# zsyOAOA/ResShift

Measured on AMD Instinct MI355X. Metric: images/sec (1x3x64x64 LR -> 3x256x256, 15-step ResShift sampling loop incl. VQ encode/decode), higher is better.
Workload: dtype f16x2 encoder + UNet (hi+lo fp16 pairs, 3 MFMAs per product: fp32-class) + f16 decoder (parity policy); 1 GPU; realsr_swinunet_realesrgan256: batch 32/GPU x 1 GPU, 1x3x64x64 LR -> 3x256x256, 15 steps, random-init weights; precision_policy=parity, parallelism=dp1 (batch sharded, one RCCL weight broadcast, no data-path collective)

## Files before the change

### include/resshift_hip.h

```cpp
#ifndef RESSHIFT_HIP_H
#define RESSHIFT_HIP_H
#include <stddef.h>
#include <stdint.h>

#ifdef __cplusplus
extern "C" {
#endif

#define RS_PREC_F16 0
#define RS_PREC_F32 1
#define RS_PREC_SPLIT 2
#define RS_MAX_LEVELS 8
#define RS_MAX_STEPS 64
#define RS_MAX_ROWS 64

typedef struct rs_engine rs_engine;

typedef struct rs_unet_config {
    int image_size, in_channels, model_channels, out_channels;
    int n_levels;
    int channel_mult[RS_MAX_LEVELS];
    int num_res_blocks[RS_MAX_LEVELS];
    int n_attn_res;
    int attention_resolutions[RS_MAX_LEVELS];
// ... 136 lines not shown
int rs_op_groupnorm(const void* x, void* y, const float* gamma_host, const float* beta_host, const float* film_dev, int B, int HW,
                    int C, int groups, float eps, int act, int prec, void* stream);
int rs_op_window_attention(const void* qkv, void* out, const float* bias_table_host , int B, int H, int W,
                           int heads, int shift, int prec, void* stream);
int rs_op_window_attention_qkv(const void* x, const void* wqkv_dev, const float* bqkv_dev, const void* wproj_dev, const float* bproj_dev,
                               const void* res, void* out, const float* table_host, int B, int H, int W, int heads, int shift, void* stream);
int rs_op_window_attention_qkv_split(const void* x, const void* wqkv_dev, const float* bqkv_dev, const void* wproj_dev, const float* bproj_dev,
                                     const void* res, void* out, const float* table_host, const float* xcoef_dev, int B, int H, int W, int heads,
                                     int shift, void* stream);
int rs_op_ae_flash_attention(const void* q, const void* k, const void* vt, const float* bv_dev, void* o, int nz, int T, int C, void* stream);
int rs_op_ae_flash_attention_split(const void* q, const void* k, const void* vt, const float* bv_dev, void* o, int nz, int T, int C, void* stream);
int rs_op_swin_mlp(const void* x, const void* w1_dev, const float* b1_dev, const void* w2_dev, const float* b2_dev, const void* res, void* y,
                   int M, int E, int HD, void* stream);
int rs_op_swin_mlp_split(const void* x, const void* w1_dev, const float* b1_dev, const void* w2_dev, const float* b2_dev, const void* res, void* y,
                         int M, int E, int HD, void* stream);
int rs_op_swin_mlp_split_unembed(const void* x, const float* xcoef_dev, const void* w1_dev, const float* b1_dev, const void* w2cat_dev, const float* bcat_dev,
                                 void* y, int M, int HW, int E, int HD, int NO, void* stream);
int rs_op_softmax_rows(const float* s, void* out, long long nrows, int ncols, int out_prec, void* stream);
int rs_op_vq(const float* z, const float* codebook_dev, float* zq, int32_t* idx, long long N, int NE, int D, void* stream);
int rs_op_nchw_to_nhwc(const float* in, void* out, int B, int C, int HW, int out_prec, void* stream);
int rs_op_nhwc_to_nchw(const void* in, float* out, int B, int C, int HW, int in_prec, void* stream);
int rs_op_convert(const void* src, int src_prec, void* dst, int dst_prec, int C, long long npix, void* stream);

#ifdef __cplusplus
}
#endif
#endif
```

### resshift_amd/_lib.py

```python
from __future__ import annotations

import ctypes as C
import os

import torch

HERE = os.path.dirname(os.path.abspath(__file__))
LIB_PATH = os.environ.get("RESSHIFT_HIP_LIB") or os.path.join(HERE, "libresshift_hip.so")

RS_PREC_F16 = 0
RS_PREC_F32 = 1
RS_PREC_SPLIT = 2
RS_MAX_LEVELS = 8
RS_MAX_STEPS = 64
RS_MAX_ROWS = 64


class UNetConfig(C.Structure):
    _fields_ = [
        ("image_size", C.c_int), ("in_channels", C.c_int), ("model_channels", C.c_int), ("out_channels", C.c_int),
        ("n_levels", C.c_int),
        ("channel_mult", C.c_int * RS_MAX_LEVELS),
        ("num_res_blocks", C.c_int * RS_MAX_LEVELS),
        ("n_attn_res", C.c_int),
# ... 110 lines not shown
    "rs_debug_fetch_rows": (_I, [_P, _I, _I, _I, _P, _P]),
    "rs_op_conv2d": (_I, [_P, _P, _P, _P, _P, _P] + [_I] * 18 + [_P]),
    "rs_op_conv2d_bench": (_I, [_P, _P, _P, _P, _P] + [_I] * 16 + [C.POINTER(C.c_float), _P]),
    "rs_op_conv3x3_halo_stats_px": (_I, [_I, _I, _I, _I, _I, _I]),
    "rs_op_conv3x3_halo": (_I, [_P, _P, _I, _P, _P, _P, _P, _I, _I, _I, _I, _I, _I, _P, _P]),
    "rs_op_conv3x3_wino": (_I, [_P, _P, _I, _P, _P, _P, _P, _I, _I, _I, _I, _I, _P, _I, C.POINTER(C.c_float), _P]),
    "rs_op_gemm_nt": (_I, [_P, _P, _P, _P, _I, _I, _I, _I, _F, _I, _I, _P]),
    "rs_op_groupnorm": (_I, [_P, _P, _P, _P, _P, _I, _I, _I, _I, _F, _I, _I, _P]),
    "rs_op_window_attention": (_I, [_P, _P, _P, _I, _I, _I, _I, _I, _I, _P]),
    "rs_op_window_attention_qkv": (_I, [_P, _P, _P, _P, _P, _P, _P, _P, _I, _I, _I, _I, _I, _P]),
    "rs_op_window_attention_qkv_split": (_I, [_P, _P, _P, _P, _P, _P, _P, _P, _P, _I, _I, _I, _I, _I, _P]),
    "rs_op_swin_mlp": (_I, [_P, _P, _P, _P, _P, _P, _P, _I, _I, _I, _P]),
    "rs_op_ae_flash_attention": (_I, [_P, _P, _P, _P, _P, _I, _I, _I, _P]),
    "rs_op_ae_flash_attention_split": (_I, [_P, _P, _P, _P, _P, _I, _I, _I, _P]),
    "rs_op_swin_mlp_split": (_I, [_P, _P, _P, _P, _P, _P, _P, _I, _I, _I, _P]),
    "rs_op_swin_mlp_split_unembed": (_I, [_P, _P, _P, _P, _P, _P, _P, _I, _I, _I, _I, _I, _P]),
    "rs_op_softmax_rows": (_I, [_P, _P, _LL, _I, _I, _P]),
    "rs_op_vq": (_I, [_P, _P, _P, _P, _LL, _I, _I, _P]),
    "rs_op_nchw_to_nhwc": (_I, [_P, _P, _I, _I, _I, _I, _P]),
    "rs_op_nhwc_to_nchw": (_I, [_P, _P, _I, _I, _I, _I, _P]),
    "rs_op_convert": (_I, [_P, _I, _P, _I, _I, _LL, _P]),
}

_lib = None


def load() -> C.CDLL:
    global _lib
    if _lib is not None:
        return _lib
# ... 91 lines not shown
```

### resshift_amd/csrc/engine.hip

```cpp
#include "common.h"
#include "../../include/resshift_hip.h"
#include <dlfcn.h>
#include <algorithm>
#include <array>
#include <cmath>
#include <cstdio>
#include <cstring>
#include <functional>
#include <map>
#include <string>
#include <unordered_map>
#include <vector>

extern "C" {
int rs_igemm_launch(const IGemmParams* p, int in_dt, int out_dt, int nz, hipStream_t st);
int rs_igemm_splitk_plan(int M, int Cout, int Ktot, int in_dt);
int rs_igemm4_pick(const IGemmParams* p, int in_dt, int out_dt, int nz, int* TW, int* BC);
int rs_igemm4_plan(const IGemmParams* p, int in_dt, int out_dt, int nz, int* TW, int* BC, int* SEG, int* SK);
int rs_igemm4_stats_px(const IGemmParams* p, int in_dt);
int rs_wino_plan(const IGemmParams* p, int in_dt, int out_dt, int nz);
int rs_wino_launch(const IGemmParams* p, hipStream_t st);
size_t rs_wino_weight_bytes(int Cin, int Cout);
float rs_wino_pack(const float* w_ref, int Cin, int Cout, void* dst);
int rs_wino_stats_px();
// ... 2588 lines not shown
    return rc;
}

int rs_op_swin_mlp(const void* x, const void* w1_dev, const float* b1_dev, const void* w2_dev, const float* b2_dev, const void* res, void* y,
                   int M, int E, int HD, void* stream) {
    const int rc = rs_swin_mlp_launch(x, w1_dev, b1_dev, w2_dev, b2_dev, res, y, M, E, E, E, E, HD, nullptr, 0, nullptr, 0, (hipStream_t)stream);
    if (rc) fail("swin_mlp launch rejected the shape (fp16, E = 192, HD = 768 only)");
    return rc;
}
int rs_op_swin_mlp_split(const void* x, const void* w1_dev, const float* b1_dev, const void* w2_dev, const float* b2_dev, const void* res, void* y,
                         int M, int E, int HD, void* stream) {
    const int rc = rs_swin_mlp_split_launch(x, w1_dev, b1_dev, w2_dev, b2_dev, res, y, M, E, E, E, E, HD, nullptr, 0, nullptr, 0, nullptr, (hipStream_t)stream);
    if (rc) fail("swin_mlp_split launch rejected the shape (split storage, E = 192, HD = 768 only)");
    return rc;
}
int rs_op_swin_mlp_split_unembed(const void* x, const float* xcoef_dev, const void* w1_dev, const float* b1_dev, const void* w2cat_dev, const float* bcat_dev,
                                 void* y, int M, int HW, int E, int HD, int NO, void* stream) {
    const int rc = rs_swin_mlp_split_launch_n(x, w1_dev, b1_dev, w2cat_dev, bcat_dev, nullptr, y, M, E, 0, NO, E, HD, NO, xcoef_dev, HW, nullptr, 0, nullptr,
                                              (hipStream_t)stream);
    if (rc) fail("swin_mlp_split (+ patch_unembed) launch rejected the shape (split storage, E = 192, HD = 768, NO = 160, HW % 128 == 0 only)");
    return rc;
}
int rs_op_softmax_rows(const float* s, void* out, long long nrows, int ncols, int out_prec, void* stream) {
    return rs_softmax_rows_launch(s, out, out_prec, nrows, ncols, ncols, ncols, (hipStream_t)stream);
}
int rs_op_vq(const float* z, const float* codebook_dev, float* zq, int32_t* idx, long long N, int NE, int D, void* stream) {
    return rs_vq_launch(z, codebook_dev, zq, idx, N, NE, D, (hipStream_t)stream);
}
int rs_op_nchw_to_nhwc(const float* in, void* out, int B, int C, int HW, int out_prec, void* stream) {
    return rs_nchw_to_nhwc_launch(in, out, out_prec, B, C, HW, C, 0, 1.f, (hipStream_t)stream);
// ... 10 lines not shown
```

### resshift_amd/csrc/swin_mlp.hip

```cpp
#include "igemm_common.h"
#include "gn_tail.h"
#include <type_traits>
#include <cstdlib>

namespace {

using namespace igemm_detail;

typedef __attribute__((address_space(3))) void* lds_ptr_t;

__device__ __forceinline__ void lds_dma16(__amdgpu_buffer_rsrc_t r, char* lds, unsigned voff) {
    __builtin_amdgcn_raw_ptr_buffer_load_lds(r, (lds_ptr_t)lds, 16, voff, 0, 0, 0);
}

template <int FC2>
__device__ __forceinline__ void mlp_stats(const f32x4 (&o)[FC2][2], float* ystats, int ld, int mw, int HW, int c0, int lr, int lg) {
    const int b = mw / HW, slab = (mw - b * HW) >> 5;
    float* dst = ystats + (((long long)b * (HW >> 5) + slab) * ld + c0) * 2;
#pragma unroll
    for (int i = 0; i < FC2; ++i)
#pragma unroll
        for (int r = 0; r < 4; ++r) {
            const float a = rs_sum16(o[i][0][r] + o[i][1][r]), q = rs_sum16(fmaf(o[i][0][r], o[i][0][r], o[i][1][r] * o[i][1][r]));
            if (lr == 0) { dst[(i * 16 + lg * 4 + r) * 2] = a; dst[(i * 16 + lg * 4 + r) * 2 + 1] = q; }
        }
}

#ifdef RS_SPLIT_ABLATE
__device__ long long g_mlp_clk[8 * 4096];
#define RS_MLP_STAMP(k) do { __builtin_amdgcn_sched_barrier(0); if (tid == 0 && blockIdx.x < 4096) g_mlp_clk[8 * blockIdx.x + (k)] = clock64(); } while (0)
#else
#define RS_MLP_STAMP(k)
#endif

struct MlpParams {
    const f16* x; const f16* w1; const float* b1; const f16* w2; const float* b2; const f16* res; f16* y;
    int M, ldx, ldres, ldy;
    const float* xcoef;
    int HW;
    float* ystats;
    int ystats_ld;
};

template <int E, int HD>
__global__ __launch_bounds__(512, 2) void swin_mlp_kernel(MlpParams p) {
    constexpr int BP = 128, HC = 64, NHC = HD / HC, KS1 = E / 64, NSL = 3;
    constexpr int W1R = 0, W1_STAGE = HC * 128, W1_SLOT = KS1 * W1_STAGE;
// ... 196 lines not shown
    return hipGetLastError() == hipSuccess ? 0 : -1;
}

namespace {

struct MlpSplitParams {
    const f16* x; const f16* w1; const float* b1; const f16* w2; const float* b2; const f16* res; f16* y;
    int M, ldx, ldres, ldy;
    const float* xcoef;
    int HW;
    float* ystats;
    int ystats_ld;
    GNTail tail;
};

template <int E, int HD, int NO = E>
__global__ __launch_bounds__(512, 2) void swin_mlp_split_kernel(MlpSplitParams p) {
    constexpr bool FOLD = NO != E;
    constexpr int BP = 128, HS = 32, NST = HD / HS, KC = E / 32;
    constexpr int NSTT = FOLD ? NST + KC : NST, HDT = FOLD ? HD + E : HD;
    constexpr int W1_SLOT = KC * HS * 128, W2_SLOT = NO * 128;
    constexpr int W1R = 0, W2R = 2 * W1_SLOT, PS = W2R + 2 * W2_SLOT;
    constexpr int FC2 = NO / 32;
    static_assert(E % 64 == 0 && NO % 32 == 0 && NO <= E && HD % HS == 0 && PS + BP * 128 <= 160 * 1024, "shape");

    extern __shared__ __attribute__((aligned(16))) char smem[];
    const int tid = threadIdx.x, lane = tid & 63;
    const int wave = __builtin_amdgcn_readfirstlane(tid >> 6);
    const int lr = lane & 15, lg = lane >> 4;
    const int wp = wave & 3, wc = wave >> 2;
    const int kcp = (lane & 7) ^ ((lane >> 3) & 7);
    const int m0 = blockIdx.x * BP;

    const __amdgpu_buffer_rsrc_t r1 = __builtin_amdgcn_make_buffer_rsrc((void*)p.w1, 0, (unsigned)(HD * E * 4), 0x00020000);
    const __amdgpu_buffer_rsrc_t r2 = __builtin_amdgcn_make_buffer_rsrc((void*)p.w2, 0, (unsigned)(HDT * NO * 4), 0x00020000);
    auto issue_w = [&](int t, int slot) {
        const unsigned plane = (unsigned)(kcp >> 2), sub = (unsigned)(kcp & 3) * 8u;
        if (!FOLD || t < NST) {
#pragma unroll
            for (int q = 0; q < 3; ++q) {
                const int piece = wave * 3 + q;
                const int c = piece >> 2, rg = piece & 3;
                const unsigned n = (unsigned)(t * HS + rg * 8 + (lane >> 3));
                lds_dma16(r1, smem + W1R + slot * W1_SLOT + piece * 1024, (n * (unsigned)(2 * E) + plane * (unsigned)E + (unsigned)(c * 32) + sub) * 2u);
            }
        }
#pragma unroll
        for (int q = 0; q < 3; ++q) {
            const int piece = wave * 3 + q;
            if (NO < 192 && piece * 8 >= NO) continue;
            const unsigned n = (unsigned)(piece * 8 + (lane >> 3));
            lds_dma16(r2, smem + W2R + slot * W2_SLOT + piece * 1024, (n * (unsigned)(2 * HDT) + plane * (unsigned)HDT + (unsigned)(t * HS) + sub) * 2u);
        }
    };
    RS_MLP_STAMP(0);
    issue_w(0, 0);

    f16x8 xh[KC][2], xl[KC][2];
#pragma unroll
    for (int j = 0; j < 2; ++j) {
        const int m = min(m0 + wp * 32 + j * 16 + lr, p.M - 1);
        const f16* xr = p.x + (long long)m * p.ldx * 2 + lg * 8;
#pragma unroll
        for (int c = 0; c < KC; ++c) { xh[c][j] = *(const f16x8*)(xr + c * 32); xl[c][j] = *(const f16x8*)(xr + p.ldx + c * 32); }
    }
    if (p.xcoef) {
        const float* sc = p.xcoef + (long long)(m0 / p.HW) * 2 * E;
#pragma unroll
        for (int c = 0; c < KC; ++c) {
            const int c0 = c * 32 + lg * 8;
            const f32x4 a0 = *(const f32x4*)(sc + c0), a1 = *(const f32x4*)(sc + c0 + 4);
            const f32x4 d0 = *(const f32x4*)(sc + E + c0), d1 = *(const f32x4*)(sc + E + c0 + 4);
#pragma unroll
            for (int j = 0; j < 2; ++j)
#pragma unroll
                for (int e = 0; e < 8; ++e) {
                    f16 hh, ll;
                    rs_split(fmaf(rs_join(xh[c][j][e], xl[c][j][e]), e < 4 ? a0[e & 3] : a1[e & 3], e < 4 ? d0[e & 3] : d1[e & 3]), hh, ll);
                    xh[c][j][e] = hh; xl[c][j][e] = ll;
                }
        }
    }
    const int swh = (lg ^ (lr & 7)) << 4, swl = ((4 + lg) ^ (lr & 7)) << 4;
    f32x4 o[FC2][2];
#pragma unroll
    for (int i = 0; i < FC2; ++i) { o[i][0] = f32x4{0.f, 0.f, 0.f, 0.f}; o[i][1] = f32x4{0.f, 0.f, 0.f, 0.f}; }

    RS_MLP_STAMP(1);
    for (int t = 0; t < NST; ++t) {
        const int slot = t & 1;
        asm volatile("s_waitcnt vmcnt(0)" ::: "memory");
        __builtin_amdgcn_s_barrier();
        if (t + 1 < NSTT) issue_w(t + 1, slot ^ 1);
        const f32x4 bv = *(const f32x4*)(p.b1 + t * HS + wc * 16 + lg * 4);
        f32x4 s_[2] = {f32x4{0.f, 0.f, 0.f, 0.f}, f32x4{0.f, 0.f, 0.f, 0.f}};
#pragma unroll
        for (int c = 0; c < KC; ++c) {
            const char* pa = smem + W1R + slot * W1_SLOT + c * (HS * 128) + (wc * 16 + lr) * 128;
            const f16x8 ah = *(const f16x8*)(pa + swh), al = *(const f16x8*)(pa + swl);
            const f16x8 as = ah * (f16)RS_LO_SCALE;
#pragma unroll
            for (int j = 0; j < 2; ++j) {
                s_[j] = __builtin_amdgcn_mfma_f32_16x16x32_f16(as, xh[c][j], s_[j], 0, 0, 0);
                s_[j] = __builtin_amdgcn_mfma_f32_16x16x32_f16(ah, xl[c][j], s_[j], 0, 0, 0);
                s_[j] = __builtin_amdgcn_mfma_f32_16x16x32_f16(al, xh[c][j], s_[j], 0, 0, 0);
            }
        }
        if (FOLD && t == NST - 1) {
#pragma unroll
            for (int j = 0; j < 2; ++j) {
                const int m = min(m0 + wp * 32 + j * 16 + lr, p.M - 1);
                const f16* xr = p.x + (long long)m * p.ldx * 2 + lg * 8;
#pragma unroll
                for (int c = 0; c < KC; ++c) { xh[c][j] = *(const f16x8*)(xr + c * 32); xl[c][j] = *(const f16x8*)(xr + p.ldx + c * 32); }
            }
        }
        {
            const int h = wc * 16 + lg * 4;
#pragma unroll
            for (int j = 0; j < 2; ++j) {
                const int m = wp * 32 + j * 16 + lr;
                rs_f16x2 h0, l0, h1, l1;
                rs_split2(rs_gelu_acc2(__builtin_elementwise_fma(rs_f32x2{s_[j][0], s_[j][1]}, rs_f32x2{RS_LO_INV, RS_LO_INV}, rs_f32x2{bv[0], bv[1]})), h0, l0);
                rs_split2(rs_gelu_acc2(__builtin_elementwise_fma(rs_f32x2{s_[j][2], s_[j][3]}, rs_f32x2{RS_LO_INV, RS_LO_INV}, rs_f32x2{bv[2], bv[3]})), h1, l1);
                char* row = smem + PS + m * 128 + (h & 7) * 2;
                *(f16x4*)(row + (((h >> 3) ^ (m & 7)) << 4)) = f16x4{h0.x, h0.y, h1.x, h1.y};
                *(f16x4*)(row + (((4 + (h >> 3)) ^ (m & 7)) << 4)) = f16x4{l0.x, l0.y, l1.x, l1.y};
            }
        }
        asm volatile("s_waitcnt lgkmcnt(0)" ::: "memory");
        __builtin_amdgcn_s_barrier();
        {
            const char* pa = smem + W2R + slot * W2_SLOT + (wc * (NO / 2) + lr) * 128;
            const char* pb = smem + PS + (wp * 32 + lr) * 128;
            f16x8 bh[2], bl[2];
#pragma unroll
            for (int j = 0; j < 2; ++j) { bh[j] = *(const f16x8*)(pb + j * 2048 + swh); bl[j] = *(const f16x8*)(pb + j * 2048 + swl); }
#pragma unroll
            for (int i = 0; i < FC2; ++i) {
                const f16x8 ah = *(const f16x8*)(pa + i * 2048 + swh), al = *(const f16x8*)(pa + i * 2048 + swl);
                const f16x8 as = ah * (f16)RS_LO_SCALE;
#pragma unroll
                for (int j = 0; j < 2; ++j) {
                    o[i][j] = __builtin_amdgcn_mfma_f32_16x16x32_f16(as, bh[j], o[i][j], 0, 0, 0);
                    o[i][j] = __builtin_amdgcn_mfma_f32_16x16x32_f16(ah, bl[j], o[i][j], 0, 0, 0);
                    o[i][j] = __builtin_amdgcn_mfma_f32_16x16x32_f16(al, bh[j], o[i][j], 0, 0, 0);
                }
            }
        }
#ifdef RS_SPLIT_ABLATE
        if (t == 0) RS_MLP_STAMP(2);
#endif
    }
    if constexpr (FOLD) {
#pragma unroll
        for (int c = 0; c < KC; ++c) {
            const int t = NST + c, slot = t & 1;
            asm volatile("s_waitcnt vmcnt(0)" ::: "memory");
            __builtin_amdgcn_s_barrier();
            if (t + 1 < NSTT) issue_w(t + 1, slot ^ 1);
            const char* pa = smem + W2R + slot * W2_SLOT + (wc * (NO / 2) + lr) * 128;
#pragma unroll
            for (int i = 0; i < FC2; ++i) {
                const f16x8 ah = *(const f16x8*)(pa + i * 2048 + swh), al = *(const f16x8*)(pa + i * 2048 + swl);
                const f16x8 as = ah * (f16)RS_LO_SCALE;
#pragma unroll
                for (int j = 0; j < 2; ++j) {
                    o[i][j] = __builtin_amdgcn_mfma_f32_16x16x32_f16(as, xh[c][j], o[i][j], 0, 0, 0);
                    o[i][j] = __builtin_amdgcn_mfma_f32_16x16x32_f16(ah, xl[c][j], o[i][j], 0, 0, 0);
                    o[i][j] = __builtin_amdgcn_mfma_f32_16x16x32_f16(al, xh[c][j], o[i][j], 0, 0, 0);
                }
            }
        }
    }
    RS_MLP_STAMP(3);
    __syncthreads();
    RS_MLP_STAMP(4);

    constexpr int ROWB = (NO / 2) * 2 + 16;
    char* stg = smem + wave * 32 * ROWB;
    const bool res_ok = !FOLD && p.res != nullptr;
    f16x4 rh[FC2][2], rl[FC2][2];
    if (res_ok) {
#pragma unroll
        for (int j = 0; j < 2; ++j) {
            const long long mr = (long long)min(m0 + wp * 32 + j * 16 + lr, p.M - 1) * p.ldres * 2;
#pragma unroll
            for (int i = 0; i < FC2; ++i) {
                const int n = wc * (NO / 2) + i * 16 + lg * 4;
                rh[i][j] = *(const f16x4*)(p.res + mr + n); rl[i][j] = *(const f16x4*)(p.res + mr + p.ldres + n);
            }
        }
    }
#pragma unroll
    for (int i = 0; i < FC2; ++i) {
        const int n = wc * (NO / 2) + i * 16 + lg * 4;
        const f32x4 bv = *(const f32x4*)(p.b2 + n);
#pragma unroll
        for (int j = 0; j < 2; ++j) {
            f32x4 v = o[i][j] * RS_LO_INV + bv;
            if (res_ok) {
#pragma unroll
                for (int r = 0; r < 4; ++r) v[r] += rs_join(rh[i][j][r], rl[i][j][r]);
            }
            o[i][j] = v;
        }
    }
    float* const sb = (float*)(smem + 8 * 32 * ROWB);
    unsigned* const tail_flag = (unsigned*)(sb + 8 * (NO / 2) * 2);
    const bool tail_on = p.ystats != nullptr && p.tail.coef != nullptr;
    const int img = m0 / (p.HW > 0 ? p.HW : 1);
    if (p.ystats) {
#pragma unroll
        for (int i = 0; i < FC2; ++i)
#pragma unroll
            for (int r = 0; r < 4; ++r) {
                const float a = rs_sum16(o[i][0][r] + o[i][1][r]), q = rs_sum16(fmaf(o[i][0][r], o[i][0][r], o[i][1][r] * o[i][1][r]));
                if (lr == 0) { sb[(wave * (NO / 2) + i * 16 + lg * 4 + r) * 2] = a; sb[(wave * (NO / 2) + i * 16 + lg * 4 + r) * 2 + 1] = q; }
            }
        __syncthreads();
        if (wave == 0) {
            float* dst = p.ystats + (((long long)img * (p.HW >> 7) + ((m0 - img * p.HW) >> 7)) * p.ystats_ld) * 2;
            for (int c = lane; c < NO; c += 64) {
                const int hw_ = c / (NO / 2), cl = c - hw_ * (NO / 2);
                float a = 0.f, q = 0.f;
#pragma unroll
                for (int w4 = 0; w4 < 4; ++w4) { a += sb[((hw_ * 4 + w4) * (NO / 2) + cl) * 2]; q += sb[((hw_ * 4 + w4) * (NO / 2) + cl) * 2 + 1]; }
                if (tail_on) rs_pub_pair(dst + c * 2, a, q);
                else { dst[c * 2] = a; dst[c * 2 + 1] = q; }
            }
            if (tail_on) { const bool last = rs_gn_tail_arrive(p.tail, img); if (lane == 0) *tail_flag = last ? 1u : 0u; }
        }
    }
    RS_MLP_STAMP(5);
    constexpr int CPR = (NO / 2) / 8, NITEM = 32 * CPR;
#pragma unroll
    for (int half = 0; half < 2; ++half) {
#pragma unroll
        for (int i = 0; i < FC2; ++i)
#pragma unroll
            for (int j = 0; j < 2; ++j) {
                f16x4 h;
#pragma unroll
                for (int r = 0; r < 4; ++r) { f16 hh, ll; rs_split(o[i][j][r], hh, ll); h[r] = half ? ll : hh; }
                *(f16x4*)(stg + (j * 16 + lr) * ROWB + (i * 16 + lg * 4) * 2) = h;
            }
        RS_STAGING_SYNC();
        for (int idx = lane; idx < NITEM; idx += 64) {
            const int row = idx / CPR, c8 = idx - row * CPR;
            const int m = m0 + wp * 32 + row;
            if (m >= p.M) continue;
            *(uint4*)(p.y + (long long)m * p.ldy * 2 + half * p.ldy + wc * (NO / 2) + c8 * 8) = *(const uint4*)(stg + row * ROWB + c8 * 16);
        }
        RS_STAGING_SYNC();
    }
    RS_MLP_STAMP(6);
    if (tail_on) {
        __syncthreads();
        if (*tail_flag) rs_gn_tail_finish<512>(p.tail, img, (float*)smem);
    }
}

}

#ifdef RS_SPLIT_ABLATE
extern "C" int rs_mlp_phase_cycles(int nwg, double* out6) {
    static long long h[8 * 4096];
    if (nwg < 1 || nwg > 4096) return -1;
    (void)hipDeviceSynchronize();
    if (hipMemcpyFromSymbol(h, HIP_SYMBOL(g_mlp_clk), sizeof(long long) * 8 * nwg) != hipSuccess) return -1;
    for (int k = 0; k < 6; ++k) {
        out6[k] = 0.0;
        for (int i = 0; i < nwg; ++i) out6[k] += (double)(h[8 * i + k + 1] - h[8 * i + k]) / nwg;
    }
    return 0;
}
#endif

extern "C" int rs_swin_mlp_split_unembed_supported(int E, int HD, int NO) { return E == 192 && HD == 768 && NO == 160; }

extern "C" int rs_swin_mlp_split_launch_n(const void* x, const void* w1, const float* b1, const void* w2, const float* b2, const void* res, void* y,
                                          int M, int ldx, int ldres, int ldy, int E, int HD, int NO, const float* xcoef, int HW, float* ystats,
                                          int ystats_ld, const GNTail* tail, hipStream_t st) {
    if (NO <= 0) NO = E;
    if (ystats && (HW <= 0 || (HW & 127) || (M & 127))) return -2;
    if (tail && tail->coef && !ystats) return -2;
    if (!rs_swin_mlp_supported(E, HD) || (ldx & 7) || (ldy & 7) || (res && (ldres & 3)) || M <= 0) return -2;
    if (NO != E && (!rs_swin_mlp_split_unembed_supported(E, HD, NO) || res || !xcoef)) return -2;
    if (xcoef && (HW <= 0 || HW % 128)) return -2;
    MlpSplitParams p{};
    p.x = (const f16*)x; p.w1 = (const f16*)w1; p.b1 = b1; p.w2 = (const f16*)w2; p.b2 = b2; p.res = (const f16*)res; p.y = (f16*)y;
    p.M = M; p.ldx = ldx; p.ldres = ldres; p.ldy = ldy; p.xcoef = xcoef; p.HW = HW; p.ystats = ystats; p.ystats_ld = ystats_ld;
    if (tail && tail->coef) {
        p.tail = *tail;
        p.tail.expected = HW / 128;
        p.tail.st0 = ystats; p.tail.S0 = HW / 128; p.tail.ld0 = ystats_ld; p.tail.n0 = NO;
    }
    constexpr int LDS = 2 * 6 * 32 * 128 + 2 * 192 * 128 + 128 * 128;
    static RsAttrFlags attr_flags;
    if (attr_flags.need()) {
        (void)hipFuncSetAttribute((const void*)swin_mlp_split_kernel<192, 768>, hipFuncAttributeMaxDynamicSharedMemorySize, LDS);
        (void)hipFuncSetAttribute((const void*)swin_mlp_split_kernel<192, 768, 160>, hipFuncAttributeMaxDynamicSharedMemorySize, LDS);
    }
    if (NO == 160) hipLaunchKernelGGL((swin_mlp_split_kernel<192, 768, 160>), dim3((M + 127) / 128), dim3(512), LDS, st, p);
    else hipLaunchKernelGGL((swin_mlp_split_kernel<192, 768>), dim3((M + 127) / 128), dim3(512), LDS, st, p);
    return hipGetLastError() == hipSuccess ? 0 : -1;
}

extern "C" int rs_swin_mlp_split_launch(const void* x, const void* w1, const float* b1, const void* w2, const float* b2, const void* res, void* y,
                                        int M, int ldx, int ldres, int ldy, int E, int HD, const float* xcoef, int HW, float* ystats, int ystats_ld,
                                        const GNTail* tail, hipStream_t st) {
    return rs_swin_mlp_split_launch_n(x, w1, b1, w2, b2, res, y, M, ldx, ldres, ldy, E, HD, E, xcoef, HW, ystats, ystats_ld, tail, st);
}
// ... 1 lines not shown
```

### resshift_amd/ops.py

```python
from __future__ import annotations

import ctypes as C

import torch

from . import _lib

F16, F32, SPLIT = _lib.RS_PREC_F16, _lib.RS_PREC_F32, _lib.RS_PREC_SPLIT


def _dt(prec: int) -> torch.dtype:
    return {F16: torch.float16, F32: torch.float32, SPLIT: torch.int32}[prec]


def _prec_of(t: torch.Tensor) -> int:
    return {torch.float16: F16, torch.float32: F32, torch.int32: SPLIT}[t.dtype]


def convert(x, prec):
    lib = _lib.load()
    x = x.contiguous()
    Cc = x.shape[-1]
    out = torch.empty(x.shape, device=x.device, dtype=_dt(prec))
    _lib.check(lib.rs_op_convert(x.data_ptr(), _prec_of(x), out.data_ptr(), prec, Cc, x.numel() // Cc, _lib.current_stream_ptr()), "convert")
# ... 161 lines not shown
    bd = bv.to(q.device, torch.float32).contiguous() if bv is not None else None
    o = torch.empty(nz, T, C, device=q.device, dtype=torch.int32)
    rc = lib.rs_op_ae_flash_attention_split(qs.data_ptr(), ks.data_ptr(), vts.data_ptr(), bd.data_ptr() if bd is not None else None, o.data_ptr(),
                                            nz, T, C, _lib.current_stream_ptr())
    _lib.check(rc, "rs_op_ae_flash_attention_split")
    return o


def split_pack_rows(w):
    w = w.detach().float()
    hi = w.half()
    lo = ((w - hi.float()) * 2048.0).half()
    return torch.cat([hi, lo], dim=1).contiguous()


def swin_mlp(x, w1, b1, w2, b2, res=None):
    lib = _lib.load()
    M, E = x.shape
    HD = w1.shape[0]
    split = x.dtype == torch.int32
    if split:
        w1d, w2d = split_pack_rows(w1).to(x.device), split_pack_rows(w2).to(x.device)
    else:
        w1d, w2d = w1.to(x.device, torch.float16).contiguous(), w2.to(x.device, torch.float16).contiguous()
    b1d, b2d = b1.to(x.device, torch.float32).contiguous(), b2.to(x.device, torch.float32).contiguous()
    y = torch.empty(M, E, device=x.device, dtype=x.dtype)
    fn = lib.rs_op_swin_mlp_split if split else lib.rs_op_swin_mlp
    rc = fn(x.data_ptr(), w1d.data_ptr(), b1d.data_ptr(), w2d.data_ptr(), b2d.data_ptr(), res.data_ptr() if res is not None else None,
            y.data_ptr(), M, E, HD, _lib.current_stream_ptr())
    _lib.check(rc, "swin_mlp")
    return y


def swin_mlp_unembed(x, coef, hw, w1, b1, w2, b2, wu, bu):
    lib = _lib.load()
    M, E = x.shape
    HD, NO = w1.shape[0], wu.shape[0]
    wcat = torch.cat([wu.double() @ w2.double(), wu.double()], dim=1).float()
    bcat = (wu.double() @ b2.double() + bu.double()).float()
    w1d, wcd = split_pack_rows(w1).to(x.device), split_pack_rows(wcat).to(x.device)
    b1d, bcd = b1.to(x.device, torch.float32).contiguous(), bcat.to(x.device).contiguous()
# ... 63 lines not shown
```

Before: 133.6 images/sec.

## Restructure split Swin MLP kernel: per-wave token rows, triple-buffered weights, interleaved GEMMs

Reworks the split-precision Swin MLP kernel so each wave owns 16 tokens across all output columns instead of a 4x2 wave grid. It also replaces double buffering with a three-slot weight ring whose DMA is waited on by counted vmcnt, and overlaps the next step's first GEMM with the GELU of the current step. This removes the LDS round-trip for the hidden activation and one barrier per step, and it caches b1 in LDS. It adds a scale-choice branch based on the input magnitude, a stats-returning entry point and ablation timers. The cost is more LDS and register pressure, and the interleave is hard-coded for six K chunks.

```diff
diff --git a/include/resshift_hip.h b/include/resshift_hip.h
--- a/include/resshift_hip.h
+++ b/include/resshift_hip.h
@@ -174,6 +174,8 @@
                    int M, int E, int HD, void* stream);
 int rs_op_swin_mlp_split(const void* x, const void* w1_dev, const float* b1_dev, const void* w2_dev, const float* b2_dev, const void* res, void* y,
                          int M, int E, int HD, void* stream);
+int rs_op_swin_mlp_split_stats(const void* x, const void* w1_dev, const float* b1_dev, const void* w2_dev, const float* b2_dev, const void* res, void* y,
+                               float* ystats, int M, int HW, int E, int HD, void* stream);
 int rs_op_swin_mlp_split_unembed(const void* x, const float* xcoef_dev, const void* w1_dev, const float* b1_dev, const void* w2cat_dev, const float* bcat_dev,
                                  void* y, int M, int HW, int E, int HD, int NO, void* stream);
 int rs_op_softmax_rows(const float* s, void* out, long long nrows, int ncols, int out_prec, void* stream);
diff --git a/resshift_amd/_lib.py b/resshift_amd/_lib.py
--- a/resshift_amd/_lib.py
+++ b/resshift_amd/_lib.py
@@ -148,6 +148,7 @@
     "rs_op_ae_flash_attention": (_I, [_P, _P, _P, _P, _P, _I, _I, _I, _P]),
     "rs_op_ae_flash_attention_split": (_I, [_P, _P, _P, _P, _P, _I, _I, _I, _P]),
     "rs_op_swin_mlp_split": (_I, [_P, _P, _P, _P, _P, _P, _P, _I, _I, _I, _P]),
+    "rs_op_swin_mlp_split_stats": (_I, [_P, _P, _P, _P, _P, _P, _P, _P, _I, _I, _I, _I, _P]),
     "rs_op_swin_mlp_split_unembed": (_I, [_P, _P, _P, _P, _P, _P, _P, _I, _I, _I, _I, _I, _P]),
     "rs_op_softmax_rows": (_I, [_P, _P, _LL, _I, _I, _P]),
     "rs_op_vq": (_I, [_P, _P, _P, _P, _LL, _I, _I, _P]),
diff --git a/resshift_amd/csrc/engine.hip b/resshift_amd/csrc/engine.hip
--- a/resshift_amd/csrc/engine.hip
+++ b/resshift_amd/csrc/engine.hip
@@ -2626,6 +2626,12 @@
     if (rc) fail("swin_mlp_split launch rejected the shape (split storage, E = 192, HD = 768 only)");
     return rc;
 }
+int rs_op_swin_mlp_split_stats(const void* x, const void* w1_dev, const float* b1_dev, const void* w2_dev, const float* b2_dev, const void* res, void* y,
+                               float* ystats, int M, int HW, int E, int HD, void* stream) {
+    const int rc = rs_swin_mlp_split_launch(x, w1_dev, b1_dev, w2_dev, b2_dev, res, y, M, E, E, E, E, HD, nullptr, HW, ystats, E, nullptr, (hipStream_t)stream);
+    if (rc) fail("swin_mlp_split launch with statistics rejected the shape (split storage, E = 192, HD = 768, HW % 128 == 0, M % 128 == 0 only)");
+    return rc;
+}
 int rs_op_swin_mlp_split_unembed(const void* x, const float* xcoef_dev, const void* w1_dev, const float* b1_dev, const void* w2cat_dev, const float* bcat_dev,
                                  void* y, int M, int HW, int E, int HD, int NO, void* stream) {
     const int rc = rs_swin_mlp_split_launch_n(x, w1_dev, b1_dev, w2cat_dev, bcat_dev, nullptr, y, M, E, 0, NO, E, HD, NO, xcoef_dev, HW, nullptr, 0, nullptr,
diff --git a/resshift_amd/csrc/swin_mlp.hip b/resshift_amd/csrc/swin_mlp.hip
--- a/resshift_amd/csrc/swin_mlp.hip
+++ b/resshift_amd/csrc/swin_mlp.hip
@@ -29,8 +29,11 @@
 #ifdef RS_SPLIT_ABLATE
 __device__ long long g_mlp_clk[8 * 4096];
 #define RS_MLP_STAMP(k) do { __builtin_amdgcn_sched_barrier(0); if (tid == 0 && blockIdx.x < 4096) g_mlp_clk[8 * blockIdx.x + (k)] = clock64(); } while (0)
+__device__ long long g_mlp_step[4 * 4096];
+#define RS_MLP_STEP_T(k) do { __builtin_amdgcn_sched_barrier(0); const long long c_ = clock64(); stp[k] += c_ - stp_last; stp_last = c_; } while (0)
 #else
 #define RS_MLP_STAMP(k)
+#define RS_MLP_STEP_T(k)
 #endif
 
 struct MlpParams {
@@ -257,56 +260,74 @@
     GNTail tail;
 };
 
+__device__ __forceinline__ void mlp_wait_vm(int n) {
+    if (n >= 6) asm volatile("s_waitcnt vmcnt(6)" ::: "memory");
+    else if (n == 5) asm volatile("s_waitcnt vmcnt(5)" ::: "memory");
+    else if (n >= 3) asm volatile("s_waitcnt vmcnt(3)" ::: "memory");
+    else if (n == 2) asm volatile("s_waitcnt vmcnt(2)" ::: "memory");
+    else asm volatile("s_waitcnt vmcnt(0)" ::: "memory");
+}
+
 template <int E, int HD, int NO = E>
 __global__ __launch_bounds__(512, 2) void swin_mlp_split_kernel(MlpSplitParams p) {
     constexpr bool FOLD = NO != E;
     constexpr int BP = 128, HS = 32, NST = HD / HS, KC = E / 32;
     constexpr int NSTT = FOLD ? NST + KC : NST, HDT = FOLD ? HD + E : HD;
     constexpr int W1_SLOT = KC * HS * 128, W2_SLOT = NO * 128;
-    constexpr int W1R = 0, W2R = 2 * W1_SLOT, PS = W2R + 2 * W2_SLOT;
-    constexpr int FC2 = NO / 32;
-    static_assert(E % 64 == 0 && NO % 32 == 0 && NO <= E && HD % HS == 0 && PS + BP * 128 <= 160 * 1024, "shape");
+    constexpr int NSLOT = 3, W2R = NSLOT * W1_SLOT, B1S = W2R + NSLOT * W2_SLOT;
+    constexpr int NF = NO / 16;
+    static_assert(E % 32 == 0 && NO % 16 == 0 && NO <= E && HD % HS == 0 && HD % 4 == 0 && HD / 4 <= 512 && NST >= 3 && B1S + HD * 4 <= 160 * 1024, "shape");
 
     extern __shared__ __attribute__((aligned(16))) char smem[];
     const int tid = threadIdx.x, lane = tid & 63;
     const int wave = __builtin_amdgcn_readfirstlane(tid >> 6);
     const int lr = lane & 15, lg = lane >> 4;
-    const int wp = wave & 3, wc = wave >> 2;
     const int kcp = (lane & 7) ^ ((lane >> 3) & 7);
     const int m0 = blockIdx.x * BP;
+    const int nw2 = min(3, max(0, NO / 8 - wave * 3));
 
     const __amdgpu_buffer_rsrc_t r1 = __builtin_amdgcn_make_buffer_rsrc((void*)p.w1, 0, (unsigned)(HD * E * 4), 0x00020000);
     const __amdgpu_buffer_rsrc_t r2 = __builtin_amdgcn_make_buffer_rsrc((void*)p.w2, 0, (unsigned)(HDT * NO * 4), 0x00020000);
-    auto issue_w = [&](int t, int slot) {
-        const unsigned plane = (unsigned)(kcp >> 2), sub = (unsigned)(kcp & 3) * 8u;
-        if (!FOLD || t < NST) {
-#pragma unroll
-            for (int q = 0; q < 3; ++q) {
-                const int piece = wave * 3 + q;
-                const int c = piece >> 2, rg = piece & 3;
-                const unsigned n = (unsigned)(t * HS + rg * 8 + (lane >> 3));
-                lds_dma16(r1, smem + W1R + slot * W1_SLOT + piece * 1024, (n * (unsigned)(2 * E) + plane * (unsigned)E + (unsigned)(c * 32) + sub) * 2u);
-            }
-        }
+    const unsigned plane = (unsigned)(kcp >> 2), sub = (unsigned)(kcp & 3) * 8u;
+    auto issue_w1 = [&](int t, int slot) {
 #pragma unroll
         for (int q = 0; q < 3; ++q) {
             const int piece = wave * 3 + q;
-            if (NO < 192 && piece * 8 >= NO) continue;
+            const int c = piece >> 2, rg = piece & 3;
+            const int r8 = lane >> 3;
+            const unsigned n = (unsigned)(t * HS + (((rg & 1) * 2 + (r8 >> 2)) * 8 + (rg >> 1) * 4 + (r8 & 3)));
+            lds_dma16(r1, smem + slot * W1_SLOT + piece * 1024, (n * (unsigned)(2 * E) + plane * (unsigned)E + (unsigned)(c * 32) + sub) * 2u);
+        }
+    };
+    auto issue_w2 = [&](int t, int slot) {
+#pragma unroll
+        for (int q = 0; q < 3; ++q) {
+            const int piece = wave * 3 + q;
+            if (q >= nw2) continue;
             const unsigned n = (unsigned)(piece * 8 + (lane >> 3));
             lds_dma16(r2, smem + W2R + slot * W2_SLOT + piece * 1024, (n * (unsigned)(2 * HDT) + plane * (unsigned)HDT + (unsigned)(t * HS) + sub) * 2u);
         }
     };
+    auto request = [&](int t, int s2) {
+        if (t + 3 < NST) issue_w1(t + 3, s2);
+        if (t + 2 < NSTT) issue_w2(t + 2, s2 == 0 ? 2 : s2 - 1);
+    };
+    auto n_request = [&](int t) { return (t + 3 < NST ? 3 : 0) + (t + 2 < NSTT ? nw2 : 0); };
     RS_MLP_STAMP(0);
-    issue_w(0, 0);
-
-    f16x8 xh[KC][2], xl[KC][2];
-#pragma unroll
-    for (int j = 0; j < 2; ++j) {
-        const int m = min(m0 + wp * 32 + j * 16 + lr, p.M - 1);
-        const f16* xr = p.x + (long long)m * p.ldx * 2 + lg * 8;
-#pragma unroll
-        for (int c = 0; c < KC; ++c) { xh[c][j] = *(const f16x8*)(xr + c * 32); xl[c][j] = *(const f16x8*)(xr + p.ldx + c * 32); }
-    }
+    f32x4 b1v = f32x4{0.f, 0.f, 0.f, 0.f};
+    if (tid < HD / 4) b1v = *(const f32x4*)(p.b1 + tid * 4);
+    issue_w1(0, 0);
+
+    f16x8 xh[KC], xl[KC];
+    const int mtok = min(m0 + wave * 16 + lr, p.M - 1);
+    {
+        const f16* xr = p.x + (long long)mtok * p.ldx * 2 + lg * 8;
+#pragma unroll
+        for (int c = 0; c < KC; ++c) { xh[c] = *(const f16x8*)(xr + c * 32); xl[c] = *(const f16x8*)(xr + p.ldx + c * 32); }
+    }
+    issue_w1(1, 1); issue_w2(0, 0);
+    issue_w1(2, 2); issue_w2(1, 1);
+    if (tid < HD / 4) *(f32x4*)(smem + B1S + tid * 16) = b1v;
     if (p.xcoef) {
         const float* sc = p.xcoef + (long long)(m0 / p.HW) * 2 * E;
 #pragma unroll
@@ -315,160 +336,186 @@
             const f32x4 a0 = *(const f32x4*)(sc + c0), a1 = *(const f32x4*)(sc + c0 + 4);
             const f32x4 d0 = *(const f32x4*)(sc + E + c0), d1 = *(const f32x4*)(sc + E + c0 + 4);
 #pragma unroll
-            for (int j = 0; j < 2; ++j)
-#pragma unroll
-                for (int e = 0; e < 8; ++e) {
-                    f16 hh, ll;
-                    rs_split(fmaf(rs_join(xh[c][j][e], xl[c][j][e]), e < 4 ? a0[e & 3] : a1[e & 3], e < 4 ? d0[e & 3] : d1[e & 3]), hh, ll);
-                    xh[c][j][e] = hh; xl[c][j][e] = ll;
-                }
+            for (int e = 0; e < 8; ++e) {
+                f16 hh, ll;
+                rs_split(fmaf(rs_join(xh[c][e], xl[c][e]), e < 4 ? a0[e & 3] : a1[e & 3], e < 4 ? d0[e & 3] : d1[e & 3]), hh, ll);
+                xh[c][e] = hh; xl[c][e] = ll;
+            }
         }
     }
     const int swh = (lg ^ (lr & 7)) << 4, swl = ((4 + lg) ^ (lr & 7)) << 4;
-    f32x4 o[FC2][2];
-#pragma unroll
-    for (int i = 0; i < FC2; ++i) { o[i][0] = f32x4{0.f, 0.f, 0.f, 0.f}; o[i][1] = f32x4{0.f, 0.f, 0.f, 0.f}; }
+    f32x4 o[NF];
+#pragma unroll
+    for (int i = 0; i < NF; ++i) o[i] = f32x4{0.f, 0.f, 0.f, 0.f};
+
+    f16x8 xs[KC];
+    float xmax = 0.f;
+#pragma unroll
+    for (int c = 0; c < KC; ++c) {
+        xs[c] = xh[c] * (f16)RS_LO_SCALE;
+#pragma unroll
+        for (int e = 0; e < 8; ++e) xmax = fmaxf(xmax, fabsf((float)xh[c][e]));
+    }
+    const bool xbig = __builtin_amdgcn_ballot_w64(!(xmax < 31.5f)) != 0;
+    using ScaleW = std::true_type; using ScaleB = std::false_type;
+    auto gemm1_chunk = [&](auto sw, const char* w1s, int c, f32x4 (&s)[2]) {
+        constexpr bool SW = decltype(sw)::value;
+        const char* pa = w1s + c * (HS * 128);
+        f16x8 ah[2], al[2], a0[2];
+#pragma unroll
+        for (int f = 0; f < 2; ++f) {
+            ah[f] = *(const f16x8*)(pa + f * 2048 + swh); al[f] = *(const f16x8*)(pa + f * 2048 + swl);
+            a0[f] = SW ? ah[f] * (f16)RS_LO_SCALE : ah[f];
+        }
+#pragma unroll
+        for (int f = 0; f < 2; ++f) s[f] = __builtin_amdgcn_mfma_f32_16x16x32_f16(a0[f], SW ? xh[c] : xs[c], s[f], 0, 0, 0);
+#pragma unroll
+        for (int f = 0; f < 2; ++f) s[f] = __builtin_amdgcn_mfma_f32_16x16x32_f16(ah[f], xl[c], s[f], 0, 0, 0);
+#pragma unroll
+        for (int f = 0; f < 2; ++f) s[f] = __builtin_amdgcn_mfma_f32_16x16x32_f16(al[f], xh[c], s[f], 0, 0, 0);
+    };
+    auto act2 = [&](float s0, float s1, float c0, float c1, rs_f16x2& h, rs_f16x2& l, float& m) {
+        const rs_f32x2 v = rs_gelu_acc2(__builtin_elementwise_fma(rs_f32x2{s0, s1}, rs_f32x2{RS_LO_INV, RS_LO_INV}, rs_f32x2{c0, c1}));
+        m = fmaxf(m, fmaxf(fabsf(v.x), fabsf(v.y)));
+        rs_split2(v, h, l);
+    };
+    auto gemm2 = [&](auto sw, const char* w2s, const f16x8& bh, const f16x8& bl) {
+        constexpr bool SW = decltype(sw)::value;
+        const f16x8 bs = SW ? bh : bh * (f16)RS_LO_SCALE;
+#pragma unroll
+        for (int i = 0; i < NF; ++i) {
+            const f16x8 ah = *(const f16x8*)(w2s + i * 2048 + swh), al = *(const f16x8*)(w2s + i * 2048 + swl);
+            const f16x8 a0 = SW ? ah * (f16)RS_LO_SCALE : ah;
+            o[i] = __builtin_amdgcn_mfma_f32_16x16x32_f16(a0, bs, o[i], 0, 0, 0);
+            o[i] = __builtin_amdgcn_mfma_f32_16x16x32_f16(ah, bl, o[i], 0, 0, 0);
+            o[i] = __builtin_amdgcn_mfma_f32_16x16x32_f16(al, bh, o[i], 0, 0, 0);
+        }
+    };
+
+    asm volatile("s_waitcnt vmcnt(0) lgkmcnt(0)" ::: "memory");
+    __builtin_amdgcn_s_barrier();
+    f32x4 s_[2] = {f32x4{0.f, 0.f, 0.f, 0.f}, f32x4{0.f, 0.f, 0.f, 0.f}};
+    if (xbig) {
+#pragma unroll
+        for (int c = 0; c < KC; ++c) gemm1_chunk(ScaleW{}, smem + lr * 128, c, s_);
+    } else {
+#pragma unroll
+        for (int c = 0; c < KC; ++c) gemm1_chunk(ScaleB{}, smem + lr * 128, c, s_);
+    }
 
     RS_MLP_STAMP(1);
+#ifdef RS_SPLIT_ABLATE
+    long long stp[4] = {0, 0, 0, 0}, stp_last = clock64();
+#endif
+    int s2 = 0;
     for (int t = 0; t < NST; ++t) {
-        const int slot = t & 1;
-        asm volatile("s_waitcnt vmcnt(0)" ::: "memory");
+        mlp_wait_vm(n_request(t - 1));
         __builtin_amdgcn_s_barrier();
-        if (t + 1 < NSTT) issue_w(t + 1, slot ^ 1);
-        const f32x4 bv = *(const f32x4*)(p.b1 + t * HS + wc * 16 + lg * 4);
-        f32x4 s_[2] = {f32x4{0.f, 0.f, 0.f, 0.f}, f32x4{0.f, 0.f, 0.f, 0.f}};
-#pragma unroll
-        for (int c = 0; c < KC; ++c) {
-            const char* pa = smem + W1R + slot * W1_SLOT + c * (HS * 128) + (wc * 16 + lr) * 128;
-            const f16x8 ah = *(const f16x8*)(pa + swh), al = *(const f16x8*)(pa + swl);
-            const f16x8 as = ah * (f16)RS_LO_SCALE;
-#pragma unroll
-            for (int j = 0; j < 2; ++j) {
-                s_[j] = __builtin_amdgcn_mfma_f32_16x16x32_f16(as, xh[c][j], s_[j], 0, 0, 0);
-                s_[j] = __builtin_amdgcn_mfma_f32_16x16x32_f16(ah, xl[c][j], s_[j], 0, 0, 0);
-                s_[j] = __builtin_amdgcn_mfma_f32_16x16x32_f16(al, xh[c][j], s_[j], 0, 0, 0);
+        RS_MLP_STEP_T(0);
+        const f32x4 bv0 = *(const f32x4*)(smem + B1S + (t * HS + lg * 8) * 4), bv1 = *(const f32x4*)(smem + B1S + (t * HS + lg * 8 + 4) * 4);
+        rs_f16x2 h0, l0, h1, l1, h2, l2, h3, l3;
+        float hmax = 0.f;
+        f32x4 sn[2] = {f32x4{0.f, 0.f, 0.f, 0.f}, f32x4{0.f, 0.f, 0.f, 0.f}};
+        auto gemm1_and_act = [&](auto sw) {
+            const char* const w1s = smem + (s2 == 2 ? 0 : s2 + 1) * W1_SLOT + lr * 128;
+            gemm1_chunk(sw, w1s, 0, sn);
+            act2(s_[0][0], s_[0][1], bv0[0], bv0[1], h0, l0, hmax);
+            gemm1_chunk(sw, w1s, 1, sn);
+            act2(s_[0][2], s_[0][3], bv0[2], bv0[3], h1, l1, hmax);
+            gemm1_chunk(sw, w1s, 2, sn);
+            act2(s_[1][0], s_[1][1], bv1[0], bv1[1], h2, l2, hmax);
+            gemm1_chunk(sw, w1s, 3, sn);
+            act2(s_[1][2], s_[1][3], bv1[2], bv1[3], h3, l3, hmax);
+            gemm1_chunk(sw, w1s, 4, sn);
+            gemm1_chunk(sw, w1s, 5, sn);
+            static_assert(KC == 6, "the interleave above is written for six chunks");
+        };
+        if (t + 1 < NST) {
+            if (xbig) gemm1_and_act(ScaleW{});
+            else gemm1_and_act(ScaleB{});
+            if (FOLD && t + 1 == NST - 1) {
+                const f16* xr = p.x + (long long)mtok * p.ldx * 2 + lg * 8;
+#pragma unroll
+                for (int c = 0; c < KC; ++c) { xh[c] = *(const f16x8*)(xr + c * 32); xl[c] = *(const f16x8*)(xr + p.ldx + c * 32); }
             }
-        }
-        if (FOLD && t == NST - 1) {
-#pragma unroll
-            for (int j = 0; j < 2; ++j) {
-                const int m = min(m0 + wp * 32 + j * 16 + lr, p.M - 1);
-                const f16* xr = p.x + (long long)m * p.ldx * 2 + lg * 8;
-#pragma unroll
-                for (int c = 0; c < KC; ++c) { xh[c][j] = *(const f16x8*)(xr + c * 32); xl[c][j] = *(const f16x8*)(xr + p.ldx + c * 32); }
-            }
-        }
-        {
-            const int h = wc * 16 + lg * 4;
-#pragma unroll
-            for (int j = 0; j < 2; ++j) {
-                const int m = wp * 32 + j * 16 + lr;
-                rs_f16x2 h0, l0, h1, l1;
-                rs_split2(rs_gelu_acc2(__builtin_elementwise_fma(rs_f32x2{s_[j][0], s_[j][1]}, rs_f32x2{RS_LO_INV, RS_LO_INV}, rs_f32x2{bv[0], bv[1]})), h0, l0);
-                rs_split2(rs_gelu_acc2(__builtin_elementwise_fma(rs_f32x2{s_[j][2], s_[j][3]}, rs_f32x2{RS_LO_INV, RS_LO_INV}, rs_f32x2{bv[2], bv[3]})), h1, l1);
-                char* row = smem + PS + m * 128 + (h & 7) * 2;
-                *(f16x4*)(row + (((h >> 3) ^ (m & 7)) << 4)) = f16x4{h0.x, h0.y, h1.x, h1.y};
-                *(f16x4*)(row + (((4 + (h >> 3)) ^ (m & 7)) << 4)) = f16x4{l0.x, l0.y, l1.x, l1.y};
-            }
-        }
-        asm volatile("s_waitcnt lgkmcnt(0)" ::: "memory");
-        __builtin_amdgcn_s_barrier();
-        {
-            const char* pa = smem + W2R + slot * W2_SLOT + (wc * (NO / 2) + lr) * 128;
-            const char* pb = smem + PS + (wp * 32 + lr) * 128;
-            f16x8 bh[2], bl[2];
-#pragma unroll
-            for (int j = 0; j < 2; ++j) { bh[j] = *(const f16x8*)(pb + j * 2048 + swh); bl[j] = *(const f16x8*)(pb + j * 2048 + swl); }
-#pragma unroll
-            for (int i = 0; i < FC2; ++i) {
-                const f16x8 ah = *(const f16x8*)(pa + i * 2048 + swh), al = *(const f16x8*)(pa + i * 2048 + swl);
-                const f16x8 as = ah * (f16)RS_LO_SCALE;
-#pragma unroll
-                for (int j = 0; j < 2; ++j) {
-                    o[i][j] = __builtin_amdgcn_mfma_f32_16x16x32_f16(as, bh[j], o[i][j], 0, 0, 0);
-                    o[i][j] = __builtin_amdgcn_mfma_f32_16x16x32_f16(ah, bl[j], o[i][j], 0, 0, 0);
-                    o[i][j] = __builtin_amdgcn_mfma_f32_16x16x32_f16(al, bh[j], o[i][j], 0, 0, 0);
-                }
-            }
-        }
+        } else {
+            act2(s_[0][0], s_[0][1], bv0[0], bv0[1], h0, l0, hmax);
+            act2(s_[0][2], s_[0][3], bv0[2], bv0[3], h1, l1, hmax);
+            act2(s_[1][0], s_[1][1], bv1[0], bv1[1], h2, l2, hmax);
+            act2(s_[1][2], s_[1][3], bv1[2], bv1[3], h3, l3, hmax);
+        }
+        const f16x8 bh = f16x8{h0.x, h0.y, h1.x, h1.y, h2.x, h2.y, h3.x, h3.y}, bl = f16x8{l0.x, l0.y, l1.x, l1.y, l2.x, l2.y, l3.x, l3.y};
+        request(t, s2);
+        RS_MLP_STEP_T(1);
+        if (__builtin_amdgcn_ballot_w64(!(hmax < 31.5f)) != 0) gemm2(ScaleW{}, smem + W2R + s2 * W2_SLOT + lr * 128, bh, bl);
+        else gemm2(ScaleB{}, smem + W2R + s2 * W2_SLOT + lr * 128, bh, bl);
+        s_[0] = sn[0]; s_[1] = sn[1];
+        s2 = s2 == NSLOT - 1 ? 0 : s2 + 1;
+        RS_MLP_STEP_T(2);
 #ifdef RS_SPLIT_ABLATE
         if (t == 0) RS_MLP_STAMP(2);
 #endif
     }
+#ifdef RS_SPLIT_ABLATE
+    if (tid == 0 && blockIdx.x < 4096)
+        for (int k = 0; k < 4; ++k) g_mlp_step[4 * blockIdx.x + k] = stp[k];
+#endif
     if constexpr (FOLD) {
 #pragma unroll
         for (int c = 0; c < KC; ++c) {
-            const int t = NST + c, slot = t & 1;
+            const int t = NST + c;
             asm volatile("s_waitcnt vmcnt(0)" ::: "memory");
             __builtin_amdgcn_s_barrier();
-            if (t + 1 < NSTT) issue_w(t + 1, slot ^ 1);
-            const char* pa = smem + W2R + slot * W2_SLOT + (wc * (NO / 2) + lr) * 128;
-#pragma unroll
-            for (int i = 0; i < FC2; ++i) {
-                const f16x8 ah = *(const f16x8*)(pa + i * 2048 + swh), al = *(const f16x8*)(pa + i * 2048 + swl);
-                const f16x8 as = ah * (f16)RS_LO_SCALE;
-#pragma unroll
-                for (int j = 0; j < 2; ++j) {
-                    o[i][j] = __builtin_amdgcn_mfma_f32_16x16x32_f16(as, xh[c][j], o[i][j], 0, 0, 0);
-                    o[i][j] = __builtin_amdgcn_mfma_f32_16x16x32_f16(ah, xl[c][j], o[i][j], 0, 0, 0);
-                    o[i][j] = __builtin_amdgcn_mfma_f32_16x16x32_f16(al, xh[c][j], o[i][j], 0, 0, 0);
-                }
-            }
+            request(t, s2);
+            gemm2(ScaleW{}, smem + W2R + s2 * W2_SLOT + lr * 128, xh[c], xl[c]);
+            s2 = s2 == NSLOT - 1 ? 0 : s2 + 1;
         }
     }
     RS_MLP_STAMP(3);
     __syncthreads();
     RS_MLP_STAMP(4);
 
-    constexpr int ROWB = (NO / 2) * 2 + 16;
-    char* stg = smem + wave * 32 * ROWB;
+    constexpr int ROWB = NO * 2 + 16;
+    char* stg = smem + wave * 16 * ROWB;
     const bool res_ok = !FOLD && p.res != nullptr;
-    f16x4 rh[FC2][2], rl[FC2][2];
+    f16x4 rh[NF], rl[NF];
     if (res_ok) {
-#pragma unroll
-        for (int j = 0; j < 2; ++j) {
-            const long long mr = (long long)min(m0 + wp * 32 + j * 16 + lr, p.M - 1) * p.ldres * 2;
-#pragma unroll
-            for (int i = 0; i < FC2; ++i) {
-                const int n = wc * (NO / 2) + i * 16 + lg * 4;
-                rh[i][j] = *(const f16x4*)(p.res + mr + n); rl[i][j] = *(const f16x4*)(p.res + mr + p.ldres + n);
-            }
-        }
-    }
-#pragma unroll
-    for (int i = 0; i < FC2; ++i) {
-        const int n = wc * (NO / 2) + i * 16 + lg * 4;
-        const f32x4 bv = *(const f32x4*)(p.b2 + n);
-#pragma unroll
-        for (int j = 0; j < 2; ++j) {
-            f32x4 v = o[i][j] * RS_LO_INV + bv;
-            if (res_ok) {
-#pragma unroll
-                for (int r = 0; r < 4; ++r) v[r] += rs_join(rh[i][j][r], rl[i][j][r]);
-            }
-            o[i][j] = v;
-        }
-    }
-    float* const sb = (float*)(smem + 8 * 32 * ROWB);
-    unsigned* const tail_flag = (unsigned*)(sb + 8 * (NO / 2) * 2);
+        const long long mr = (long long)mtok * p.ldres * 2;
+#pragma unroll
+        for (int i = 0; i < NF; ++i) {
+            const int n = i * 16 + lg * 4;
+            rh[i] = *(const f16x4*)(p.res + mr + n); rl[i] = *(const f16x4*)(p.res + mr + p.ldres + n);
+        }
+    }
+#pragma unroll
+    for (int i = 0; i < NF; ++i) {
+        const f32x4 bv = *(const f32x4*)(p.b2 + i * 16 + lg * 4);
+        f32x4 v = o[i] * RS_LO_INV + bv;
+        if (res_ok) {
+#pragma unroll
+            for (int r = 0; r < 4; ++r) v[r] += rs_join(rh[i][r], rl[i][r]);
+        }
+        o[i] = v;
+    }
+    float* const sb = (float*)(smem + 8 * 16 * ROWB);
+    unsigned* const tail_flag = (unsigned*)(sb + 8 * NO * 2);
     const bool tail_on = p.ystats != nullptr && p.tail.coef != nullptr;
     const int img = m0 / (p.HW > 0 ? p.HW : 1);
     if (p.ystats) {
 #pragma unroll
-        for (int i = 0; i < FC2; ++i)
+        for (int i = 0; i < NF; ++i)
 #pragma unroll
             for (int r = 0; r < 4; ++r) {
-                const float a = rs_sum16(o[i][0][r] + o[i][1][r]), q = rs_sum16(fmaf(o[i][0][r], o[i][0][r], o[i][1][r] * o[i][1][r]));
-                if (lr == 0) { sb[(wave * (NO / 2) + i * 16 + lg * 4 + r) * 2] = a; sb[(wave * (NO / 2) + i * 16 + lg * 4 + r) * 2 + 1] = q; }
+                const float a = rs_sum16(o[i][r]), q = rs_sum16(o[i][r] * o[i][r]);
+                if (lr == 0) { sb[(wave * NO + i * 16 + lg * 4 + r) * 2] = a; sb[(wave * NO + i * 16 + lg * 4 + r) * 2 + 1] = q; }
             }
         __syncthreads();
         if (wave == 0) {
             float* dst = p.ystats + (((long long)img * (p.HW >> 7) + ((m0 - img * p.HW) >> 7)) * p.ystats_ld) * 2;
             for (int c = lane; c < NO; c += 64) {
-                const int hw_ = c / (NO / 2), cl = c - hw_ * (NO / 2);
                 float a = 0.f, q = 0.f;
 #pragma unroll
-                for (int w4 = 0; w4 < 4; ++w4) { a += sb[((hw_ * 4 + w4) * (NO / 2) + cl) * 2]; q += sb[((hw_ * 4 + w4) * (NO / 2) + cl) * 2 + 1]; }
+                for (int w8 = 0; w8 < 8; ++w8) { a += sb[(w8 * NO + c) * 2]; q += sb[(w8 * NO + c) * 2 + 1]; }
                 if (tail_on) rs_pub_pair(dst + c * 2, a, q);
                 else { dst[c * 2] = a; dst[c * 2 + 1] = q; }
             }
@@ -476,24 +523,22 @@
         }
     }
     RS_MLP_STAMP(5);
-    constexpr int CPR = (NO / 2) / 8, NITEM = 32 * CPR;
+    constexpr int CPR = NO / 8, NITEM = 16 * CPR;
 #pragma unroll
     for (int half = 0; half < 2; ++half) {
 #pragma unroll
-        for (int i = 0; i < FC2; ++i)
-#pragma unroll
-            for (int j = 0; j < 2; ++j) {
-                f16x4 h;
-#pragma unroll
-                for (int r = 0; r < 4; ++r) { f16 hh, ll; rs_split(o[i][j][r], hh, ll); h[r] = half ? ll : hh; }
-                *(f16x4*)(stg + (j * 16 + lr) * ROWB + (i * 16 + lg * 4) * 2) = h;
-            }
+        for (int i = 0; i < NF; ++i) {
+            f16x4 h;
+#pragma unroll
+            for (int r = 0; r < 4; ++r) { f16 hh, ll; rs_split(o[i][r], hh, ll); h[r] = half ? ll : hh; }
+            *(f16x4*)(stg + lr * ROWB + (i * 16 + lg * 4) * 2) = h;
+        }
         RS_STAGING_SYNC();
         for (int idx = lane; idx < NITEM; idx += 64) {
             const int row = idx / CPR, c8 = idx - row * CPR;
-            const int m = m0 + wp * 32 + row;
+            const int m = m0 + wave * 16 + row;
             if (m >= p.M) continue;
-            *(uint4*)(p.y + (long long)m * p.ldy * 2 + half * p.ldy + wc * (NO / 2) + c8 * 8) = *(const uint4*)(stg + row * ROWB + c8 * 16);
+            *(uint4*)(p.y + (long long)m * p.ldy * 2 + half * p.ldy + c8 * 8) = *(const uint4*)(stg + row * ROWB + c8 * 16);
         }
         RS_STAGING_SYNC();
     }
@@ -515,6 +560,17 @@
     for (int k = 0; k < 6; ++k) {
         out6[k] = 0.0;
         for (int i = 0; i < nwg; ++i) out6[k] += (double)(h[8 * i + k + 1] - h[8 * i + k]) / nwg;
+    }
+    return 0;
+}
+extern "C" int rs_mlp_step_cycles(int nwg, int nsteps, double* out3) {
+    static long long h[4 * 4096];
+    if (nwg < 1 || nwg > 4096 || nsteps < 1) return -1;
+    (void)hipDeviceSynchronize();
+    if (hipMemcpyFromSymbol(h, HIP_SYMBOL(g_mlp_step), sizeof(long long) * 4 * nwg) != hipSuccess) return -1;
+    for (int k = 0; k < 3; ++k) {
+        out3[k] = 0.0;
+        for (int i = 0; i < nwg; ++i) out3[k] += (double)h[4 * i + k] / nwg / nsteps;
     }
     return 0;
 }
@@ -539,7 +595,7 @@
         p.tail.expected = HW / 128;
         p.tail.st0 = ystats; p.tail.S0 = HW / 128; p.tail.ld0 = ystats_ld; p.tail.n0 = NO;
     }
-    constexpr int LDS = 2 * 6 * 32 * 128 + 2 * 192 * 128 + 128 * 128;
+    constexpr int LDS = 3 * (6 * 32 * 128 + 192 * 128) + 768 * 4;
     static RsAttrFlags attr_flags;
     if (attr_flags.need()) {
         (void)hipFuncSetAttribute((const void*)swin_mlp_split_kernel<192, 768>, hipFuncAttributeMaxDynamicSharedMemorySize, LDS);
diff --git a/resshift_amd/ops.py b/resshift_amd/ops.py
--- a/resshift_amd/ops.py
+++ b/resshift_amd/ops.py
@@ -199,7 +199,7 @@
     return torch.cat([hi, lo], dim=1).contiguous()
 
 
-def swin_mlp(x, w1, b1, w2, b2, res=None):
+def swin_mlp(x, w1, b1, w2, b2, res=None, want_stats=False, hw=None):
     lib = _lib.load()
     M, E = x.shape
     HD = w1.shape[0]
@@ -210,6 +210,15 @@
         w1d, w2d = w1.to(x.device, torch.float16).contiguous(), w2.to(x.device, torch.float16).contiguous()
     b1d, b2d = b1.to(x.device, torch.float32).contiguous(), b2.to(x.device, torch.float32).contiguous()
     y = torch.empty(M, E, device=x.device, dtype=x.dtype)
+    if want_stats:
+        if not split or not hw or hw % 128 or M % hw:
+            raise RuntimeError("swin_mlp statistics need split storage and whole images of a multiple of 128 tokens")
+        st = torch.zeros(M // hw, hw // 128, E, 2, device=x.device, dtype=torch.float32)
+        rc = lib.rs_op_swin_mlp_split_stats(x.data_ptr(), w1d.data_ptr(), b1d.data_ptr(), w2d.data_ptr(), b2d.data_ptr(),
+                                            res.data_ptr() if res is not None else None, y.data_ptr(), st.data_ptr(), M, hw, E, HD,
+                                            _lib.current_stream_ptr())
+        _lib.check(rc, "swin_mlp")
+        return y, st
     fn = lib.rs_op_swin_mlp_split if split else lib.rs_op_swin_mlp
     rc = fn(x.data_ptr(), w1d.data_ptr(), b1d.data_ptr(), w2d.data_ptr(), b2d.data_ptr(), res.data_ptr() if res is not None else None,
             y.data_ptr(), M, E, HD, _lib.current_stream_ptr())
```

Measured after the change: 133.9 images/sec, median of 6. No clear change (+0.2%).
